# rhofield/rho-tts

Hardware: AMD Instinct MI355X
Metric: audio-sec/wall-sec (RTF) Qwen3-TTS-1.7B batch=32 (higher is better)
Workload: dtype bf16; 1 GPU; Qwen3-TTS-1.7B bf16, batch 32/GPU, 30-s reference clone, 10-word sentences (44 frames each), sampling=top-k 50 T 0.9, seeded synthetic weights; value counts delivered (post-processed) audio; global_batch=32, parallelism=dp1

## Files before the change

rho_tts_amd/csrc/code2wav.hip:

```cpp
#include "model_internal.h"

using namespace rtm;

extern "C" {

int64_t rt_wav_length(rt_model* m, int32_t n_frames) {
    if (!m || n_frames < 0) return -1;
    int64_t L = n_frames;
    for (int i = 0; i < m->cfg.n_upsampling; ++i) L *= m->cfg.upsampling_ratios[i];
    for (int i = 0; i < m->cfg.n_upsample_rates; ++i) L = (L - 1) * m->cfg.upsample_rates[i];
    return L > 0 ? L : 0;
}

int rt_code2wav(rt_model* m, int32_t n_items, int32_t t_max, const int32_t* h_codes, const int32_t* h_n_frames, float* d_wav,
                int64_t wav_stride, int64_t* h_wav_len) {
    if (!m || !h_codes || !h_n_frames || !d_wav || !h_wav_len) return rt_fail(m ? m->ctx : nullptr, RT_ERR_INVALID, "rt_code2wav: null argument");
    rt_ctx* ctx = m->ctx;
    CtxLock g(ctx);
    RT_HIP(ctx, hipSetDevice(ctx->device));
    if (!m->finalized) return rt_fail(ctx, RT_ERR_STATE, "rt_code2wav: model not finalized");
    const rt_model_config& c = m->cfg;
    const int B = n_items, T = t_max, Q = c.num_quantizers, Hc = c.codec_tf.hidden;
    if (B < 1 || B > c.max_batch || T < 1) return rt_fail(ctx, RT_ERR_INVALID, "rt_code2wav: n_items %d / t_max %d out of range", B, T);
    if (T > c.max_codec_frames) return rt_fail(ctx, RT_ERR_LENGTH, "rt_code2wav: length %d frames exceeds max_codec_frames %d", T, c.max_codec_frames);
// ... 77 lines not shown
        RT_TRY(pool_arr(m, (size_t)rows * cout, &xr));
        RT_TRY(planes((size_t)rows * cout, &s1));
        RT_TRY(planes((size_t)rows * cout, &s2));
        {
            GemmA a; a.ptr = s_in.hi; a.ptr_lo = s_in.lo; a.split = 1; a.M = (int64_t)B * (Tc - 1); a.Cin = cin; a.taps = 2; a.tap_stride = 1; a.tap_offset = 0;
            a.rows_out = (int)(Tc - 1); a.rows_in = (int)Tc;
            GemmEpi e; e.bias = VEC(m, bn + ".tconv_b"); e.out_f32 = xr; e.out2_hi = s1.hi; e.out2_lo = s1.lo;
            e.snake2_a = m->xvec[bn + ".u0.a1"]; e.snake2_ib = m->xvec[bn + ".u0.ib1"];
            e.ldc = (int64_t)r * cout;
            RT_TRY(launch_gemm(ctx, a, PW(m, bn + ".tconv"), e));
        }
        for (int j = 0; j < 3; ++j) {
            const std::string u = bn + ".u" + std::to_string(j);
            const int dil = j == 0 ? 1 : (j == 1 ? 3 : 9);
            GemmA a; a.ptr = s1.hi; a.ptr_lo = s1.lo; a.split = 1; a.M = rows; a.Cin = cout; a.taps = 7; a.tap_stride = dil; a.tap_offset = -6 * dil;
            a.rows_out = (int)To; a.rows_in = (int)To;
            GemmEpi e; e.bias = VEC(m, u + ".c1_b"); e.act = ACT_SNAKE; e.snake_a = VEC(m, u + ".a2"); e.snake_ib = VEC(m, u + ".ib2");
            e.out_hi = s2.hi; e.out_lo = s2.lo; e.ldc = cout;
            GemmA a2; a2.ptr = s2.hi; a2.ptr_lo = s2.lo; a2.split = 1; a2.M = rows; a2.Cin = cout;
            GemmEpi e2; e2.bias = VEC(m, u + ".c2_b"); e2.residual = xr; e2.out_f32 = xr; e2.out2_hi = s1.hi; e2.out2_lo = s1.lo; e2.ldc = cout;
            if (j < 2) { e2.snake2_a = VEC(m, bn + ".u" + std::to_string(j + 1) + ".a1"); e2.snake2_ib = VEC(m, bn + ".u" + std::to_string(j + 1) + ".ib1"); }
            else if (i + 1 < c.n_upsample_rates) { e2.snake2_a = VEC(m, "codec.b" + std::to_string(i + 1) + ".sa"); e2.snake2_ib = VEC(m, "codec.b" + std::to_string(i + 1) + ".sib"); }
            else { e2.snake2_a = VEC(m, "codec.fin_a"); e2.snake2_ib = VEC(m, "codec.fin_ib"); }
            if (conv_pair_fusable(a, PW(m, u + ".c1"), e, PW(m, u + ".c2"))) {
                e2.out2_hi = s2.hi; e2.out2_lo = s2.lo;
                RT_TRY(launch_gemm(ctx, a, PW(m, u + ".c1"), e, &PW(m, u + ".c2"), &e2));
                std::swap(s1, s2);
            } else {
                RT_TRY(launch_gemm(ctx, a, PW(m, u + ".c1"), e));
                RT_TRY(launch_gemm(ctx, a2, PW(m, u + ".c2"), e2));
            }
        }
        s_in = s1;
        Tc = To;
    }
    float* wav_tmp = nullptr;
    RT_TRY(pool_arr(m, (size_t)B * Tc, &wav_tmp));
    {
        const int cl = m->dec_ch.back();
        GemmA a; a.ptr = s_in.hi; a.ptr_lo = s_in.lo; a.split = 1; a.M = (int64_t)B * Tc; a.Cin = cl; a.taps = 7; a.tap_stride = 1; a.tap_offset = -6;
        a.rows_out = (int)Tc; a.rows_in = (int)Tc;
        if (launch_final_conv_ok(cl) && g_final_conv) {
            RT_TRY(launch_final_conv(ctx, s_in.hi, s_in.lo, B, (int)Tc, cl, VEC(m, "codec.fin_wv"), VEC(m, "codec.fin_b"), wav_tmp));
        } else {
            GemmEpi e; e.bias = VEC(m, "codec.fin_b"); e.act = ACT_CLAMP1; e.out_f32 = wav_tmp; e.ldc = 1;
            RT_TRY(launch_gemm(ctx, a, PW(m, "codec.fin_w"), e));
        }
    }
    RT_HIP(ctx, hipMemcpy2DAsync(d_wav, (size_t)wav_stride * 4, wav_tmp, (size_t)Tc * 4, (size_t)Tc * 4, B, hipMemcpyDeviceToDevice, ctx->stream));
    RT_HIP(ctx, hipStreamSynchronize(ctx->stream));
    for (int b = 0; b < B; ++b) h_wav_len[b] = rt_wav_length(m, h_n_frames[b]);
    pool_release_all(m);
    return RT_OK;
}
}
```

rho_tts_amd/csrc/debug.hip:

```cpp
#include <algorithm>
#include <vector>

#include "kernels.h"

namespace {
__global__ void k_touch(float* p, int n) {
    const int i = blockIdx.x * blockDim.x + threadIdx.x;
    if (i < n) p[i] = p[i] * 1.0001f + 1.0f;
}
template <int MODE>
__global__ void k_bench_barrier(unsigned* bar, int n, float* buf) {
    const int i = blockIdx.x * blockDim.x + threadIdx.x;
    const int j = (i + blockDim.x) % (gridDim.x * blockDim.x);
    float acc = buf[i];
    for (int e = 1; e <= n; ++e) {
        if (MODE == 2) st_agent(buf + i, acc + 1.0f); else buf[i] = acc + 1.0f;
        if (!grid_barrier<MODE>(bar, gridDim.x, (unsigned)e, 1u << 20)) return;
        acc = MODE == 2 ? ld_agent(buf + j) : buf[j];
        if (acc != (float)e && i == 0) bar[2] = 1u;
    }
    buf[i] = acc;
}
template <int P>
__global__ void k_bench_pair(unsigned* flags, int n, float* buf, unsigned* bar) {
// ... 284 lines not shown
int rt_debug_sample(rt_ctx* ctx, const float* d_logits, int32_t M, int32_t V, const rt_sampling* sp, uint64_t seed, int32_t frame,
                    int32_t group, int32_t suppress_from, int32_t allow_token, uint8_t* d_seen, int32_t* d_out) {
    if (!ctx || !d_logits || !sp || !d_out || M < 1) return rt_fail(ctx, RT_ERR_INVALID, "rt_debug_sample: null argument");
    CtxLock g(ctx);
    RT_HIP(ctx, hipSetDevice(ctx->device));
    int64_t* items = nullptr;
    RT_HIP(ctx, hipMalloc((void**)&items, (size_t)M * 8));
    hipLaunchKernelGGL(k_iota64, dim3((M + 255) / 256), dim3(256), 0, ctx->stream, items, M);
    SampleArgs a{};
    a.logits = d_logits; a.n_slabs = 1; a.M = M; a.V = V;
    a.do_sample = sp->do_sample; a.temperature = sp->temperature; a.top_k = sp->top_k; a.top_p = sp->top_p; a.rep_penalty = sp->repetition_penalty;
    a.seen = d_seen; a.suppress_from = suppress_from; a.allow_token = allow_token; a.seed = seed; a.item_ids = items; a.frame = frame; a.group = group;
    a.forced = nullptr; a.out = d_out; a.out_stride = 1; a.eos_token = -1; a.eos_flag = nullptr; a.logits_copy = nullptr;
    a.frame_ptr = nullptr; a.seed_ptr = nullptr; a.stamps = nullptr;
    int rc = launch_sample(ctx, a);
    (void)hipStreamSynchronize(ctx->stream);
    (void)hipFree(items);
    return rc;
}

int rt_debug_tune(int32_t skinny_variant, int32_t skinny_waves_per_cu) {
    std::unique_lock<std::shared_mutex> all(g_tune_mu);
    if (g_runs_in_flight.load() > 0) return RT_ERR_STATE;
    if (skinny_variant >= 2800) { g_pair_attn = skinny_variant - 2800; return RT_OK; }
    if (skinny_variant >= 2700) { g_frame_inc_fold = skinny_variant - 2700; return RT_OK; }
    if (skinny_variant >= 2600) { g_conv_unroll = skinny_variant - 2600; return RT_OK; }
    if (skinny_variant >= 2400) { g_col_silu_x = skinny_variant - 2400; return RT_OK; }
    if (skinny_variant >= 2300) { g_col_rows16 = skinny_variant - 2300; return RT_OK; }
    if (skinny_variant >= 2200) { g_prefill_attn_mfma = skinny_variant - 2200; return RT_OK; }
    if (skinny_variant >= 2100) { g_fuse_conv = skinny_variant - 2100; return RT_OK; }
    if (skinny_variant >= 2000) { g_col_max_rows = std::min(64, std::max(1, skinny_variant - 2000)); return RT_OK; }
    if (skinny_variant >= 1900) { g_prefill_mid = skinny_variant - 1900; return RT_OK; }
    if (skinny_variant >= 1800) { g_conv_tall = skinny_variant - 1800; return RT_OK; }
    if (skinny_variant >= 1700) { g_handover_every = std::max(1, skinny_variant - 1700); return RT_OK; }
    if (skinny_variant >= 1600) { g_col_split4 = skinny_variant - 1600; return RT_OK; }
    if (skinny_variant >= 1500) { g_attn_mfma = skinny_variant - 1500; return RT_OK; }
    if (skinny_variant >= 1400) { g_eos_check_every = std::max(1, skinny_variant - 1400); return RT_OK; }
    if (skinny_variant >= 1300) { g_sync_parts = skinny_variant - 1300; return RT_OK; }
    if (skinny_variant >= 1200) { g_conv_win = skinny_variant - 1200; return RT_OK; }
    if (skinny_variant >= 1100) { g_final_conv = skinny_variant - 1100; return RT_OK; }
    if (skinny_variant >= 1000) { g_xcd_order = skinny_variant - 1000; return RT_OK; }
    if (skinny_variant >= 900) { g_prefill_fill = skinny_variant - 900; return RT_OK; }
    if (skinny_variant >= 800) { g_fuse_sample_embed = skinny_variant - 800; return RT_OK; }
    if (skinny_variant >= 700) { g_col_rows64 = skinny_variant - 700; return RT_OK; }
    if (skinny_variant >= 600) { g_tile96 = skinny_variant - 600; return RT_OK; }
    if (skinny_variant >= 500) { g_col_split = skinny_variant - 500; return RT_OK; }
// ... 288 lines not shown
```

rho_tts_amd/csrc/gemm.hip:

```cpp
#include <hip/hip_ext.h>

#include "kernels.h"

namespace {

typedef __attribute__((ext_vector_type(8))) __bf16 bf8_t;
typedef __attribute__((ext_vector_type(8))) short s8_t;
typedef __attribute__((ext_vector_type(16))) float f16_t;
typedef __attribute__((ext_vector_type(4))) float f4_t;
typedef __attribute__((ext_vector_type(4))) int i4_t;

__device__ __forceinline__ f16_t mfma32(s8_t a, s8_t b, f16_t c) {
    return __builtin_amdgcn_mfma_f32_32x32x16_bf16(__builtin_bit_cast(bf8_t, a), __builtin_bit_cast(bf8_t, b), c, 0, 0, 0);
}

__device__ __forceinline__ unsigned pack_bf16x2(float lo, float hi) {
    return f32x2_to_bf16x2(lo, hi);
}

__global__ void k_pack_weight(const bf16_t* __restrict__ src, int N, int K, int Np, int Kp, bf16_t* __restrict__ dst) {
    const int KT = Kp / 16;
    const int64_t n_pieces = (int64_t)(Np / 32) * KT * 64;
    for (int64_t p = (int64_t)blockIdx.x * blockDim.x + threadIdx.x; p < n_pieces; p += (int64_t)gridDim.x * blockDim.x) {
        const int lane = (int)(p & 63);
// ... 618 lines not shown
    for (int j = 0; j < PF - 1; ++j) {
        if (it + j < n_it) {
            multiply(j & 1);
            flush();
            stash((j + 1) & 1, rg[j + 1]);
            __syncthreads();
        }
    }
#pragma unroll
    for (int a = 0; a < WM; ++a)
#pragma unroll
        for (int b = 0; b < WN; ++b) {
            const int n = n0 + (wn * WN + b) * 32 + r;
            if (n >= g.N) continue;
#pragma unroll
            for (int i = 0; i < 16; ++i) {
                const int64_t m = m0 + (wm * WM + a) * 32 + (i & 3) + 8 * (i >> 2) + 4 * h;
                if (m < g.M) g.out[m * g.ldc + n] = g.seg_it > 0 ? tot[a][b][i] : acc[a][b][i];
            }
        }
}

template <int WGM, int WGN, int MT, int NTT, bool FUSE = false, int TAPS = 0>
__global__ __launch_bounds__(256, (WGM * MT * 32 > 128) ? 2 : 3) void k_conv_win(TiledArgs g) {
    static_assert(WGM * WGN == 4, "4 waves");
    static_assert(!FUSE || (WGN == 1 && NTT == 3), "the fused 1x1 conv needs every output channel of a row in one wave");
    constexpr int BMT = WGM * MT * 32;
    constexpr int WIN_ROWS = BMT + 64;
    constexpr int NP = (WIN_ROWS * 4 + 255) / 256;
    constexpr int BNT = WGN * NTT * 32;
    constexpr int PLANE = WIN_ROWS * 64;
    constexpr int F_ROWB = NTT * 32 * 2 + 16;
    constexpr int F_WAVE = 2 * 32 * F_ROWB;
    constexpr int LDS_BYTES = (FUSE && 4 * F_WAVE > 2 * 2 * PLANE) ? 4 * F_WAVE : 2 * 2 * PLANE;
    __shared__ __attribute__((aligned(16))) unsigned char lds[LDS_BYTES];
    const int tid = threadIdx.x, lane = tid & 63, w = tid >> 6;
    const int wm = w / WGN, wn = w % WGN;
    const int r = lane & 31, h = lane >> 5;
    int64_t rt = blockIdx.x;
    int ct = blockIdx.y;
    if (g.xcd_order) {
        const int64_t L = (int64_t)blockIdx.y * gridDim.x + blockIdx.x;
        const int xcd = (int)(L & 7);
        const int64_t j = L >> 3;
        ct = (int)(j % gridDim.y);
        rt = (j / gridDim.y) * 8 + xcd;
        if (rt * BMT >= g.a.M) return;
    }
    const int64_t m0 = rt * BMT;
    const int n0 = ct * BNT;
    const int taps = TAPS > 0 ? TAPS : g.a.taps, stride = g.a.tap_stride, Cin = g.a.Cin;
    const int halo = (taps - 1) * stride, WR = BMT + halo, n_cc = Cin >> 5;
    const bf16_t* __restrict__ hi = reinterpret_cast<const bf16_t*>(g.a.ptr);
    const bf16_t* __restrict__ lo = reinterpret_cast<const bf16_t*>(g.a.ptr_lo);

    const int64_t first_row = m0 - halo > 0 ? m0 - halo : 0;
    const int skip = (int)(first_row - (m0 - halo));
// ... 33 lines not shown
    for (int nt = 0; nt < NTT; ++nt) b_off[nt] = nt_base + nt < g.NT ? (unsigned)(((nt_base + nt) * g.KT * 64 + lane) * 16) : 0x80000000u;
    auto load_b = [&](int tap, int cc, s8_t (&b)[NTT][2]) {
        const int t_k0 = (tap * Cin + cc * 32) >> 4;
#pragma unroll
        for (int nt = 0; nt < NTT; ++nt)
#pragma unroll
            for (int kk = 0; kk < 2; ++kk) b[nt][kk] = __builtin_bit_cast(s8_t, __builtin_amdgcn_raw_buffer_load_b128(rs_w, b_off[nt], (t_k0 + kk) * 1024, 0));
    };
    int t_row[MT];
#pragma unroll
    for (int mt = 0; mt < MT; ++mt) {
        const int64_t m = m0 + (wm * MT + mt) * 32 + r;
        t_row[mt] = (int)(m % g.a.rows_out);
    }

    f16_t acc[MT][NTT];
#pragma unroll
    for (int a = 0; a < MT; ++a)
#pragma unroll
        for (int b = 0; b < NTT; ++b)
#pragma unroll
            for (int i = 0; i < 16; ++i) acc[a][b][i] = 0.f;

    s8_t ra[NP], rl[NP], rb[NTT][2], rb_next[NTT][2];
    load_win(0, ra, rl);
    load_b(0, 0, rb);
    store_win(0, ra, rl);
    __syncthreads();
    for (int cc = 0; cc < n_cc; ++cc) {
        const int buf = cc & 1;
        const bool more = cc + 1 < n_cc;
        if (more) load_win(cc + 1, ra, rl);
#pragma unroll
        for (int tap = 0; tap < (TAPS > 0 ? TAPS : taps); ++tap) {
            const bool last = tap + 1 == taps;
            if (!last) load_b(tap + 1, cc, rb_next);
            else if (more) load_b(0, cc + 1, rb_next);
            const int reach = (taps - 1 - tap) * stride;
            s8_t fa[MT][2], fl[MT][2];
#pragma unroll
            for (int mt = 0; mt < MT; ++mt) {
                const int wrow = t_row[mt] >= reach ? (wm * MT + mt) * 32 + r + tap * stride : WIN_ROWS - 1;
#pragma unroll
                for (int kk = 0; kk < 2; ++kk) {
                    fa[mt][kk] = *reinterpret_cast<const s8_t*>(lds + buf * 2 * PLANE + lds_a_off(wrow, kk * 2 + h));
                    fl[mt][kk] = *reinterpret_cast<const s8_t*>(lds + buf * 2 * PLANE + PLANE + lds_a_off(wrow, kk * 2 + h));
                }
            }
#pragma unroll
            for (int kk = 0; kk < 2; ++kk)
#pragma unroll
                for (int mt = 0; mt < MT; ++mt)
#pragma unroll
                    for (int nt = 0; nt < NTT; ++nt) {
                        acc[mt][nt] = mfma32(fa[mt][kk], rb[nt][kk], acc[mt][nt]);
                        acc[mt][nt] = mfma32(fl[mt][kk], rb[nt][kk], acc[mt][nt]);
                    }
            if (!last || more) {
#pragma unroll
                for (int nt = 0; nt < NTT; ++nt)
#pragma unroll
                    for (int kk = 0; kk < 2; ++kk) rb[nt][kk] = rb_next[nt][kk];
            }
        }
        if (more) store_win(buf ^ 1, ra, rl);
        __syncthreads();
    }
    if constexpr (!FUSE) {
        tile_epilogue<MT, NTT>(g, acc, m0, n0, wm, wn, r, h);
    } else {
        unsigned char* my = lds + w * F_WAVE;
        const GemmEpi& e = g.e;
        const __amdgpu_buffer_rsrc_t rs_w2 = __builtin_amdgcn_make_buffer_rsrc((void*)g.Wp2, 0, (unsigned)((int64_t)g.NT2 * g.KT2 * 1024), 0x00020000);
        float f_bias[NTT], f_sa[NTT], f_sib[NTT];
        {
            const float* bp = e.bias ? e.bias : e.snake_a;
#pragma unroll
            for (int nt = 0; nt < NTT; ++nt) {
                const int n = nt * 32 + r;
                f_bias[nt] = bp[n];
                f_sa[nt] = e.snake_a[n];
                f_sib[nt] = e.snake_ib[n];
            }
#pragma unroll
            for (int nt = 0; nt < NTT; ++nt)
                if (!e.bias) f_bias[nt] = 0.f;
        }
        auto load_b2 = [&](int k2, s8_t (&b)[NTT]) {
#pragma unroll
            for (int nt = 0; nt < NTT; ++nt)
                b[nt] = __builtin_bit_cast(s8_t, __builtin_amdgcn_raw_buffer_load_b128(rs_w2, (unsigned)(((nt * g.KT2 + k2) * 64 + lane) * 16), 0, 0));
        };
#pragma unroll
        for (int mt = 0; mt < MT; ++mt) {
            s8_t b2[2][NTT];
            load_b2(0, b2[0]);
#pragma unroll
            for (int nt = 0; nt < NTT; ++nt) {
                const int n = nt * 32 + r;
                const float bias = f_bias[nt], sa = f_sa[nt], sib = f_sib[nt];
#pragma unroll
                for (int i = 0; i < 16; ++i) {
                    float v = acc[mt][nt][i] + bias;
                    const float sn = __sinf(v * sa);
                    v = v + sib * sn * sn;
                    const bf16_t hi = f32_to_bf16(v);
                    const bf16_t lo = f32_to_bf16(v - bf16_to_f32(hi));
                    const int row = (i & 3) + 8 * (i >> 2) + 4 * h;
                    *reinterpret_cast<bf16_t*>(my + row * F_ROWB + n * 2) = hi;
                    *reinterpret_cast<bf16_t*>(my + 32 * F_ROWB + row * F_ROWB + n * 2) = lo;
                }
            }
            f16_t acc2[1][NTT];
#pragma unroll
            for (int nt = 0; nt < NTT; ++nt)
#pragma unroll
                for (int i = 0; i < 16; ++i) acc2[0][nt][i] = 0.f;
#pragma unroll
            for (int k2 = 0; k2 < NTT * 2; ++k2) {
                if (k2 + 1 < NTT * 2) load_b2(k2 + 1, b2[(k2 + 1) & 1]);
                const s8_t a_hi = *reinterpret_cast<const s8_t*>(my + r * F_ROWB + (k2 * 16 + h * 8) * 2);
                const s8_t a_lo = *reinterpret_cast<const s8_t*>(my + 32 * F_ROWB + r * F_ROWB + (k2 * 16 + h * 8) * 2);
#pragma unroll
                for (int nt = 0; nt < NTT; ++nt) {
                    acc2[0][nt] = mfma32(a_hi, b2[k2 & 1][nt], acc2[0][nt]);
                    acc2[0][nt] = mfma32(a_lo, b2[k2 & 1][nt], acc2[0][nt]);
                }
            }
            tile_epilogue_e<1, NTT>(g.e2, g.a.M, g.N2, acc2, m0, 0, wm * MT + mt, 0, r, h);
        }
    }
}

}

size_t packed_bytes(int N, int K) {
    const size_t Np = (size_t)(N + 31) / 32 * 32, Kp = (size_t)(K + 15) / 16 * 16;
    return Np * Kp * 2;
}

size_t packed16_bytes(int N, int K) { return (size_t)((N + 15) / 16 * 16) * K * 2; }

int launch_pack_weight16(rt_ctx* ctx, const bf16_t* d_src, int N, int K, bf16_t* d_dst, PackedW* out) {
    if (K % 32) return rt_fail(ctx, RT_ERR_INVALID, "pack16: K=%d must be a multiple of 32", K);
    const int Np = (N + 15) / 16 * 16;
    const int64_t pieces = (int64_t)(Np / 16) * (K / 32) * 64;
    int64_t blocks = (pieces + 255) / 256;
    if (blocks > 4096) blocks = 4096;
    hipLaunchKernelGGL(k_pack_weight16, dim3((unsigned)blocks), dim3(256), 0, ctx->stream, d_src, N, K, Np, d_dst);
// ... 85 lines not shown

rt_knob g_prefill_mid{1};
bool gemm_mid_shape_ok(const PackedW& w) { return g_prefill_mid && w.K % MID_BK == 0 && w.K >= 128 && w.Kp == w.K; }
bool gemm_mid_ok(int M, const PackedW& w) { return gemm_mid_shape_ok(w) && M > 64 && M <= 1024; }
int launch_gemm_mid(rt_ctx* ctx, const bf16_t* A, int M, const PackedW& w, float* out, int64_t ldc) {
    if (!gemm_mid_ok(M, w)) return rt_fail(ctx, RT_ERR_INVALID, "gemm_mid: M=%d K=%d outside its range", M, w.K);
    MidArgs g{A, w.data, out, M, w.N, w.K, w.Np / 32, w.Kp / 16, ldc, 0};
    const int S = skinny_pick_split(M, w.N, w.K, ctx->n_cu);
    if (S > 1) {
        if ((g.KT / S) % (MID_BK / 16)) return rt_fail(ctx, RT_ERR_STATE, "gemm_mid: K segments of %d k-tiles are not whole 64-deep steps (K=%d, split %d)", g.KT / S, w.K, S);
        g.seg_it = (g.KT / S) / (MID_BK / 16);
    }
    const bool big = g_prefill_mid == 1 ? (int64_t)((M + 127) / 128) * ((w.N + 63) / 64) >= 3 * ctx->n_cu : g_prefill_mid == 3;
    const int bm = big ? 128 : 64;
    const int n_rt = (M + bm - 1) / bm, n_ct = (w.N + 63) / 64;
    dim3 grid(8 * ((n_ct + 7) / 8) * n_rt);
    if (big) hipLaunchKernelGGL((k_gemm_mid<2, 1, 4>), grid, dim3(256), 0, ctx->stream, g);
    else hipLaunchKernelGGL((k_gemm_mid<1, 1, 6>), grid, dim3(256), 0, ctx->stream, g);
    RT_HIP(ctx, hipGetLastError());
    return RT_OK;
}

rt_knob g_fuse_conv{1};

bool conv_pair_fusable(const GemmA& a, const PackedW& w, const GemmEpi& e, const PackedW& w2) {
    return g_fuse_conv && g_conv_win && g_tile96 && w.N == 96 && w2.N == 96 && w2.K == 96 && w2.Kp == 96 && e.act == ACT_SNAKE && a.split && !a.is_f32 && a.ptr_lo && a.taps >= 2 &&
           a.Cin % 32 == 0 && a.rows_out > 0 && a.rows_in == a.rows_out && a.tap_offset == -(a.taps - 1) * a.tap_stride && (a.taps - 1) * a.tap_stride <= 63 &&
           a.M % a.rows_out == 0;
}

int launch_gemm(rt_ctx* ctx, const GemmA& a, const PackedW& w, const GemmEpi& e, const PackedW* w2, const GemmEpi* e2) {
    if (a.M <= 0) return RT_OK;
    if (a.Cin % 8 || (int64_t)a.Cin * a.taps != w.K)
        return rt_fail(ctx, RT_ERR_INVALID, "gemm: A has taps=%d Cin=%d but W has K=%d", a.taps, a.Cin, w.K);
    if (e.split_k < 1 || (e.split_k > 1 && !e.out_f32)) return rt_fail(ctx, RT_ERR_INVALID, "gemm: bad split_k");
    TiledArgs g;
    g.a = a;
    g.Wp = w.data;
    g.N = w.N; g.K = w.K; g.NT = w.Np / 32; g.KT = w.Kp / 16;
    g.e = e;
    int per = (g.KT + e.split_k - 1) / e.split_k;
    per = (per + 1) / 2 * 2;
    g.kt_per_split = per;
    const bool narrow = g_tile96 && e.split_k == 1 && w.N % 96 == 0 && w.N % 128 != 0;
    const bool conv_win = g_conv_win && a.split && !a.is_f32 && a.ptr_lo && a.taps >= 2 && a.Cin % 32 == 0 && a.rows_out > 0 && a.rows_in == a.rows_out &&
        a.tap_offset == -(a.taps - 1) * a.tap_stride && (a.taps - 1) * a.tap_stride <= 63 && e.split_k == 1 && a.M % a.rows_out == 0;
    const bool tall = conv_win && narrow && (g_conv_tall == 2 || (g_conv_tall == 1 && a.M >= 256 * 1024));
    const int bm = tall ? 256 : BM;
    const int64_t my = (a.M + bm - 1) / bm;
    if (my > 0x7fffffff) return rt_fail(ctx, RT_ERR_LENGTH, "gemm: length %lld rows too large", (long long)a.M);
    const int bn = narrow ? 96 : BN;
    const int ny = (w.N + bn - 1) / bn;
    g.xcd_order = (g_xcd_order && e.split_k == 1 && ny > 1 && my >= 64) ? 1 : 0;
    dim3 grid((unsigned)(g.xcd_order ? (my + 7) / 8 * 8 : my), ny, e.split_k);
    if (a.split && !a.is_f32 && !a.ptr_lo) return rt_fail(ctx, RT_ERR_INVALID, "gemm: split precision needs an f32 A operand or a low plane");
    if ((e.out_hi && !e.out_lo) || (e.out2_hi && (!e.out2_lo || (e.act2 != ACT_ELU && (!e.snake2_a || !e.snake2_ib)))) ||
        ((e.out_hi || e.out2_hi) && e.split_k > 1))
        return rt_fail(ctx, RT_ERR_INVALID, "gemm: incomplete hi/lo plane output");
    if (w2) {
        if (!e2 || !conv_win || !narrow || ny != 1 || w.N != 96 || w2->N != 96 || w2->K != 96 || e.act != ACT_SNAKE || !e.snake_a || !e.snake_ib ||
            e2->split_k != 1 || e2->ldc < 96)
            return rt_fail(ctx, RT_ERR_INVALID, "gemm: this conv pair cannot be fused (96 channels, k > 1 conv with SnakeBeta, then a 96 x 96 1x1 conv)");
        g.Wp2 = w2->data; g.NT2 = w2->Np / 32; g.KT2 = w2->Kp / 16; g.N2 = w2->N; g.e2 = *e2;
        const bool t7f = a.taps == 7 && g_conv_unroll;
        if (tall && t7f) hipLaunchKernelGGL((k_conv_win<4, 1, 2, 3, true, 7>), grid, dim3(256), 0, ctx->stream, g);
        else if (tall) hipLaunchKernelGGL((k_conv_win<4, 1, 2, 3, true>), grid, dim3(256), 0, ctx->stream, g);
        else hipLaunchKernelGGL((k_conv_win<4, 1, 1, 3, true>), grid, dim3(256), 0, ctx->stream, g);
        RT_HIP(ctx, hipGetLastError());
        return RT_OK;
    }
    if (conv_win) {
        const bool t7 = a.taps == 7 && g_conv_unroll;
        if (tall && t7) hipLaunchKernelGGL((k_conv_win<4, 1, 2, 3, false, 7>), grid, dim3(256), 0, ctx->stream, g);
        else if (tall) hipLaunchKernelGGL((k_conv_win<4, 1, 2, 3>), grid, dim3(256), 0, ctx->stream, g);
        else if (narrow) hipLaunchKernelGGL((k_conv_win<4, 1, 1, 3>), grid, dim3(256), 0, ctx->stream, g);
        else if (t7) hipLaunchKernelGGL((k_conv_win<2, 2, 2, 2, false, 7>), grid, dim3(256), 0, ctx->stream, g);
        else hipLaunchKernelGGL((k_conv_win<2, 2, 2, 2>), grid, dim3(256), 0, ctx->stream, g);
        RT_HIP(ctx, hipGetLastError());
        return RT_OK;
    }
#define RT_TILED(AF, SP)                                                                                          \
    do {                                                                                                          \
        if (narrow) hipLaunchKernelGGL((k_gemm_tiled<AF, SP, 4, 1, 1, 3>), grid, dim3(256), 0, ctx->stream, g);   \
        else hipLaunchKernelGGL((k_gemm_tiled<AF, SP, 2, 2, 2, 2>), grid, dim3(256), 0, ctx->stream, g);          \
    } while (0)
    if (a.split && !a.is_f32) RT_TILED(false, true);
    else if (a.split) RT_TILED(true, true);
// ... 7 lines not shown
```

rho_tts_amd/csrc/kernels.h:

```cpp
#pragma once
#include "common.h"

struct PackedW {
    const bf16_t* data = nullptr;
    int N = 0, K = 0;
    int Np = 0, Kp = 0;
    size_t bytes() const { return (size_t)Np * Kp * 2; }
    const bf16_t* data16 = nullptr;
    int Np16 = 0;
};

struct GemmA {
    const void* ptr = nullptr;
    const void* ptr_lo = nullptr;
    int is_f32 = 0;
    int split = 0;
    int64_t M = 0;
    int Cin = 0;
    int taps = 1;
    int tap_stride = 1;
    int tap_offset = 0;
    int rows_out = 0;
    int rows_in = 0;
};
// ... 9 lines not shown
    int act = ACT_NONE;
    const float* snake_a = nullptr;
    const float* snake_ib = nullptr;
    bf16_t* out2_bf16 = nullptr;
    float* out2_f32 = nullptr;
    bf16_t* out_hi = nullptr;
    bf16_t* out_lo = nullptr;
    bf16_t* out2_hi = nullptr;
    bf16_t* out2_lo = nullptr;
    const float* snake2_a = nullptr;
    const float* snake2_ib = nullptr;
    int act2 = ACT_SNAKE;
    int64_t ldc = 0;
    int split_k = 1;
};

size_t packed_bytes(int N, int K);
int launch_pack_weight(rt_ctx* ctx, const bf16_t* d_src, int N, int K, bf16_t* d_dst, PackedW* out);
size_t packed16_bytes(int N, int K);
int launch_pack_weight16(rt_ctx* ctx, const bf16_t* d_src, int N, int K, bf16_t* d_dst, PackedW* out);
int launch_gemm(rt_ctx* ctx, const GemmA& a, const PackedW& w, const GemmEpi& e, const PackedW* w2 = nullptr, const GemmEpi* e2 = nullptr);
bool conv_pair_fusable(const GemmA& a, const PackedW& w, const GemmEpi& e, const PackedW& w2);
extern rt_knob g_fuse_conv;
extern rt_knob g_prefill_mid;
bool gemm_mid_ok(int M, const PackedW& w);
bool gemm_mid_shape_ok(const PackedW& w);
int launch_gemm_mid(rt_ctx* ctx, const bf16_t* A, int M, const PackedW& w, float* out, int64_t ldc);
int launch_gemm_skinny(rt_ctx* ctx, const bf16_t* d_a, int M, const PackedW& w, float* d_out, int64_t ldc, int split_k,
                       hipEvent_t ev_start = nullptr, hipEvent_t ev_stop = nullptr, int64_t slab_stride = 0);
int skinny_pick_split(int M, int N, int K, int n_cu);
extern rt_knob g_decode_col;
extern rt_knob g_use_graph;
extern rt_knob g_pred_nt;
extern rt_knob g_decode_lanes;
extern rt_knob g_sync_parts;
extern rt_knob g_eos_check_every;
extern rt_knob g_handover_every;
extern rt_knob g_conv_tall;
extern rt_knob g_col_max_rows;
extern rt_knob g_tile96;
extern rt_knob g_conv_win;
extern rt_knob g_conv_unroll;
extern rt_knob g_final_conv;
extern rt_knob g_xcd_order;
extern rt_knob g_prefill_fill;
extern rt_knob g_pair_attn;
// ... 137 lines not shown
    float* logits_copy;
    const int32_t* frame_ptr;
    const int32_t* frame_off;
    int64_t out_fs, eos_fs, forced_fs, copy_fs;
    int eos_live, min_frames;
    long long* stamps;
    const float* emb_table;
    int emb_H;
    const float* emb_norm_w;
    float* emb_rowsq;
    int emb_rowsq_n;
    float* emb_x_tiled;
    bf16_t* emb_a_tiled;
};
int launch_sample(rt_ctx* ctx, const SampleArgs& a);


int launch_dwconv_ln(rt_ctx* ctx, const float* x, int B, int T, int C, const float* w , const float* b,
                     const float* ln_w, const float* ln_b, float eps, float* out_f32);
int launch_code_embed_mean(rt_ctx* ctx, const bf16_t* table, int codebook, int Q, int H, const int32_t* codes ,
                           int64_t rows, float* out_f32);

bool launch_final_conv_ok(int C);
int launch_final_conv(rt_ctx* ctx, const bf16_t* hi, const bf16_t* lo, int B, int T, int C, const float* w, const float* bias, float* wav);
int launch_f32_to_bf16(rt_ctx* ctx, const float* x, int64_t n, bf16_t* out);

int launch_enc_conv0(rt_ctx* ctx, const float* pcm, int64_t T, int C, int k, const float* w , const float* bias, float* x,
                     bf16_t* hi, bf16_t* lo);
int launch_rvq(rt_ctx* ctx, const float* sem, float* aco, int T, int D, int K, int Q, const float* const* d_cbT, int32_t* codes);
int launch_stats_pool(rt_ctx* ctx, const float* x, int T, int C, float* out);
int launch_gemv_f32(rt_ctx* ctx, const float* W, const float* b, const float* x, int N, int K, int relu, float* y);
```

rho_tts_amd/csrc/rowops.hip:

```cpp
#include "kernels.h"

namespace {

typedef __attribute__((ext_vector_type(4))) float f4_t;

__device__ __forceinline__ float block_sum_f32(float v, float* sh) {
    v = wave_sum_f32(v);
    const int w = threadIdx.x >> 6, nw = (blockDim.x + 63) >> 6;
    __syncthreads();
    if ((threadIdx.x & 63) == 0) sh[w] = v;
    __syncthreads();
    float t = 0.f;
    for (int i = 0; i < nw; ++i) t += sh[i];
    return t;
}

__global__ __launch_bounds__(256) void k_add_rmsnorm(float* __restrict__ x, int H, const float* __restrict__ slabs, int n_slabs,
                                                     int64_t slab_stride, const float* __restrict__ slab_bias,
                                                     const float* __restrict__ scale, const float* __restrict__ w, float eps,
                                                     bf16_t* __restrict__ out_bf16, float* __restrict__ out_f32) {
    __shared__ float sh[4];
    constexpr int MAXV = 8;
    const int64_t row = blockIdx.x;
    const int nv = H >> 2;
// ... 373 lines not shown
    for (int c = threadIdx.x; c < C; c += 256) { const float dlt = row[c] - mean; s2 += dlt * dlt; }
    const float var = block_sum_f32(s2, sh) / (float)C;
    const float inv = rsqrtf(var + eps);
    for (int c = threadIdx.x; c < C; c += 256) out[r * C + c] = (row[c] - mean) * inv * lw[c] + lb[c];
}

__global__ __launch_bounds__(256) void k_code_embed_mean(const bf16_t* __restrict__ table, int codebook, int Q, int H,
                                                         const int32_t* __restrict__ codes, float* __restrict__ out) {
    const int64_t r = blockIdx.x;
    const float inv = 1.f / (float)Q;
    for (int i = threadIdx.x; i < H; i += 256) {
        float v = 0.f;
        for (int q = 0; q < Q; ++q) {
            int c = codes[r * Q + q];
            c = c < 0 ? 0 : (c >= codebook ? codebook - 1 : c);
            v += bf16_to_f32(table[((int64_t)q * codebook + c) * H + i]);
        }
        out[r * H + i] = v * inv;
    }
}


__global__ __launch_bounds__(256) void k_final_conv(const bf16_t* __restrict__ hi, const bf16_t* __restrict__ lo, int T, int C,
                                                    const float* __restrict__ w, const float* __restrict__ bias, float* __restrict__ wav) {
    extern __shared__ float sm[];
    const int stride = C + 1;
    float* tile = sm;
    float* wt = sm + 134 * stride;
    const int b = blockIdx.y, t0 = blockIdx.x * 128, tid = threadIdx.x;
    for (int i = tid; i < 7 * C; i += 256) wt[i] = w[i];
    const int C8 = C >> 3;
    constexpr int IT = 7;
    const int n_items = 134 * C8;
    for (int base = 0; base < n_items; base += 256 * IT) {
        uint4 h[IT], l[IT];
#pragma unroll
        for (int u = 0; u < IT; ++u) {
            int idx = base + u * 256 + tid;
            idx = idx < n_items ? idx : n_items - 1;
            const int row = idx / C8, c = (idx - row * C8) * 8;
            int t = t0 - 6 + row;
            t = t < 0 ? 0 : (t < T ? t : T - 1);
            const int64_t o = ((int64_t)b * T + t) * C + c;
            h[u] = *reinterpret_cast<const uint4*>(hi + o);
            l[u] = *reinterpret_cast<const uint4*>(lo + o);
        }
#pragma unroll
// ... 2 lines not shown
            idx = idx < n_items ? idx : n_items - 1;
            const int row = idx / C8, c = (idx - row * C8) * 8, t = t0 - 6 + row;
            const bool in = t >= 0 && t < T;
            const unsigned hw[4] = {h[u].x, h[u].y, h[u].z, h[u].w}, lw[4] = {l[u].x, l[u].y, l[u].z, l[u].w};
#pragma unroll
            for (int e = 0; e < 4; ++e) {
                const float v0 = __uint_as_float(hw[e] << 16) + __uint_as_float(lw[e] << 16);
                const float v1 = __uint_as_float(hw[e] & 0xffff0000u) + __uint_as_float(lw[e] & 0xffff0000u);
                tile[row * stride + c + 2 * e] = in ? v0 : 0.f;
                tile[row * stride + c + 2 * e + 1] = in ? v1 : 0.f;
            }
        }
    }
    __syncthreads();
    const int s = tid >> 1, half = tid & 1, ch = C >> 1;
    float acc = 0.f;
    for (int k = 0; k < 7; ++k) {
        const float* x = tile + (s + k) * stride + half * ch;
        const float* ww = wt + k * C + half * ch;
        for (int c = 0; c < ch; ++c) acc += x[c] * ww[c];
    }
    acc += __shfl_xor(acc, 1, 64);
    const int t = t0 + s;
    if (half == 0 && t < T) wav[(int64_t)b * T + t] = fminf(1.f, fmaxf(-1.f, acc + bias[0]));
}

__global__ void k_f32_to_bf16(const float* __restrict__ x, int64_t n, bf16_t* __restrict__ out) {
    for (int64_t i = (int64_t)blockIdx.x * blockDim.x + threadIdx.x; i < n; i += (int64_t)gridDim.x * blockDim.x)
        out[i] = f32_to_bf16(x[i]);
}

inline unsigned grid_for(int64_t total, int block = 256) {
    int64_t b = (total + block - 1) / block;
    if (b > 8192) b = 8192;
    if (b < 1) b = 1;
    return (unsigned)b;
}

}

int launch_add_rmsnorm(rt_ctx* ctx, float* x, int M, int H, const float* slabs, int n_slabs, const float* slab_bias,
                       const float* scale, const float* w, float eps, bf16_t* out_bf16, float* out_f32) {
    if (M <= 0) return RT_OK;
    if (H % 4 || H > 8192) return rt_fail(ctx, RT_ERR_UNSUPPORTED, "rmsnorm: hidden size %d unsupported (multiple of 4, <= 8192)", H);
    const int64_t st = (int64_t)M * H;
    if (H == 1024) hipLaunchKernelGGL(k_add_rmsnorm_v<1>, dim3(M), dim3(256), 0, ctx->stream, x, slabs, n_slabs, st, slab_bias, scale, w, eps, out_bf16, out_f32);
    else if (H == 2048) hipLaunchKernelGGL(k_add_rmsnorm_v<2>, dim3(M), dim3(256), 0, ctx->stream, x, slabs, n_slabs, st, slab_bias, scale, w, eps, out_bf16, out_f32);
// ... 88 lines not shown
    return RT_OK;
}


int launch_dwconv_ln(rt_ctx* ctx, const float* x, int B, int T, int C, const float* w, const float* b, const float* ln_w,
                     const float* ln_b, float eps, float* out_f32) {
    const int64_t rows = (int64_t)B * T;
    if (rows <= 0) return RT_OK;
    hipLaunchKernelGGL(k_dwconv_ln, dim3((unsigned)rows), dim3(256), C * sizeof(float), ctx->stream, x, T, C, w, b, ln_w, ln_b, eps, out_f32);
    RT_HIP(ctx, hipGetLastError());
    return RT_OK;
}

int launch_code_embed_mean(rt_ctx* ctx, const bf16_t* table, int codebook, int Q, int H, const int32_t* codes, int64_t rows, float* out_f32) {
    if (rows <= 0) return RT_OK;
    hipLaunchKernelGGL(k_code_embed_mean, dim3((unsigned)rows), dim3(256), 0, ctx->stream, table, codebook, Q, H, codes, out_f32);
    RT_HIP(ctx, hipGetLastError());
    return RT_OK;
}


bool launch_final_conv_ok(int C) { return C % 16 == 0 && (size_t)(134 * (C + 1) + 7 * C) * 4 <= 64 * 1024; }

int launch_final_conv(rt_ctx* ctx, const bf16_t* hi, const bf16_t* lo, int B, int T, int C, const float* w, const float* bias, float* wav) {
    if (B <= 0 || T <= 0) return RT_OK;
    if (!launch_final_conv_ok(C)) return rt_fail(ctx, RT_ERR_UNSUPPORTED, "final conv: %d channels do not fit the LDS window", C);
    const size_t lds = (size_t)(134 * (C + 1) + 7 * C) * 4;
    hipLaunchKernelGGL(k_final_conv, dim3((T + 127) / 128, B), dim3(256), lds, ctx->stream, hi, lo, T, C, w, bias, wav);
    RT_HIP(ctx, hipGetLastError());
    return RT_OK;
}

int launch_f32_to_bf16(rt_ctx* ctx, const float* x, int64_t n, bf16_t* out) {
    if (n <= 0) return RT_OK;
    hipLaunchKernelGGL(k_f32_to_bf16, dim3(grid_for(n)), dim3(256), 0, ctx->stream, x, n, out);
    RT_HIP(ctx, hipGetLastError());
    return RT_OK;
}
```

Measured before the change: 564.9 audio-s/s.

## Fuse 192-channel codec conv pairs and write final waveform directly

Extends the fused k=7 conv + SnakeBeta + 1x1 conv kernel to 192-channel decoder blocks, staging weights in double-buffered LDS and splitting the second GEMM's staging into 96-column halves. The codec's final residual unit skips writing the unused fp32 residual stream, and the final conv writes straight into the strided output buffer instead of a temp plus a 2D memcpy. This removes intermediate global round-trips and one copy in the vocoder, at the cost of higher LDS and register use (lower occupancy bound) for the new kernel variant.

```diff
diff --git a/rho_tts_amd/csrc/code2wav.hip b/rho_tts_amd/csrc/code2wav.hip
--- a/rho_tts_amd/csrc/code2wav.hip
+++ b/rho_tts_amd/csrc/code2wav.hip
@@ -123,6 +123,7 @@
             if (j < 2) { e2.snake2_a = VEC(m, bn + ".u" + std::to_string(j + 1) + ".a1"); e2.snake2_ib = VEC(m, bn + ".u" + std::to_string(j + 1) + ".ib1"); }
             else if (i + 1 < c.n_upsample_rates) { e2.snake2_a = VEC(m, "codec.b" + std::to_string(i + 1) + ".sa"); e2.snake2_ib = VEC(m, "codec.b" + std::to_string(i + 1) + ".sib"); }
             else { e2.snake2_a = VEC(m, "codec.fin_a"); e2.snake2_ib = VEC(m, "codec.fin_ib"); }
+            if (j == 2 && g_c2w_lean) e2.out_f32 = nullptr;
             if (conv_pair_fusable(a, PW(m, u + ".c1"), e, PW(m, u + ".c2"))) {
                 e2.out2_hi = s2.hi; e2.out2_lo = s2.lo;
                 RT_TRY(launch_gemm(ctx, a, PW(m, u + ".c1"), e, &PW(m, u + ".c2"), &e2));
@@ -135,20 +136,25 @@
         s_in = s1;
         Tc = To;
     }
-    float* wav_tmp = nullptr;
-    RT_TRY(pool_arr(m, (size_t)B * Tc, &wav_tmp));
     {
         const int cl = m->dec_ch.back();
-        GemmA a; a.ptr = s_in.hi; a.ptr_lo = s_in.lo; a.split = 1; a.M = (int64_t)B * Tc; a.Cin = cl; a.taps = 7; a.tap_stride = 1; a.tap_offset = -6;
-        a.rows_out = (int)Tc; a.rows_in = (int)Tc;
-        if (launch_final_conv_ok(cl) && g_final_conv) {
-            RT_TRY(launch_final_conv(ctx, s_in.hi, s_in.lo, B, (int)Tc, cl, VEC(m, "codec.fin_wv"), VEC(m, "codec.fin_b"), wav_tmp));
+        const bool own = launch_final_conv_ok(cl) && g_final_conv;
+        if (own && g_c2w_lean) {
+            RT_TRY(launch_final_conv(ctx, s_in.hi, s_in.lo, B, (int)Tc, cl, VEC(m, "codec.fin_wv"), VEC(m, "codec.fin_b"), d_wav, wav_stride));
         } else {
-            GemmEpi e; e.bias = VEC(m, "codec.fin_b"); e.act = ACT_CLAMP1; e.out_f32 = wav_tmp; e.ldc = 1;
-            RT_TRY(launch_gemm(ctx, a, PW(m, "codec.fin_w"), e));
+            float* wav_tmp = nullptr;
+            RT_TRY(pool_arr(m, (size_t)B * Tc, &wav_tmp));
+            if (own) {
+                RT_TRY(launch_final_conv(ctx, s_in.hi, s_in.lo, B, (int)Tc, cl, VEC(m, "codec.fin_wv"), VEC(m, "codec.fin_b"), wav_tmp, Tc));
+            } else {
+                GemmA a; a.ptr = s_in.hi; a.ptr_lo = s_in.lo; a.split = 1; a.M = (int64_t)B * Tc; a.Cin = cl; a.taps = 7; a.tap_stride = 1; a.tap_offset = -6;
+                a.rows_out = (int)Tc; a.rows_in = (int)Tc;
+                GemmEpi e; e.bias = VEC(m, "codec.fin_b"); e.act = ACT_CLAMP1; e.out_f32 = wav_tmp; e.ldc = 1;
+                RT_TRY(launch_gemm(ctx, a, PW(m, "codec.fin_w"), e));
+            }
+            RT_HIP(ctx, hipMemcpy2DAsync(d_wav, (size_t)wav_stride * 4, wav_tmp, (size_t)Tc * 4, (size_t)Tc * 4, B, hipMemcpyDeviceToDevice, ctx->stream));
         }
     }
-    RT_HIP(ctx, hipMemcpy2DAsync(d_wav, (size_t)wav_stride * 4, wav_tmp, (size_t)Tc * 4, (size_t)Tc * 4, B, hipMemcpyDeviceToDevice, ctx->stream));
     RT_HIP(ctx, hipStreamSynchronize(ctx->stream));
     for (int b = 0; b < B; ++b) h_wav_len[b] = rt_wav_length(m, h_n_frames[b]);
     pool_release_all(m);
diff --git a/rho_tts_amd/csrc/debug.hip b/rho_tts_amd/csrc/debug.hip
--- a/rho_tts_amd/csrc/debug.hip
+++ b/rho_tts_amd/csrc/debug.hip
@@ -330,6 +330,8 @@
 int rt_debug_tune(int32_t skinny_variant, int32_t skinny_waves_per_cu) {
     std::unique_lock<std::shared_mutex> all(g_tune_mu);
     if (g_runs_in_flight.load() > 0) return RT_ERR_STATE;
+    if (skinny_variant >= 3000) { g_fuse_conv192 = skinny_variant - 3000; return RT_OK; }
+    if (skinny_variant >= 2900) { g_c2w_lean = skinny_variant - 2900; return RT_OK; }
     if (skinny_variant >= 2800) { g_pair_attn = skinny_variant - 2800; return RT_OK; }
     if (skinny_variant >= 2700) { g_frame_inc_fold = skinny_variant - 2700; return RT_OK; }
     if (skinny_variant >= 2600) { g_conv_unroll = skinny_variant - 2600; return RT_OK; }
diff --git a/rho_tts_amd/csrc/gemm.hip b/rho_tts_amd/csrc/gemm.hip
--- a/rho_tts_amd/csrc/gemm.hip
+++ b/rho_tts_amd/csrc/gemm.hip
@@ -664,17 +664,22 @@
 }
 
 template <int WGM, int WGN, int MT, int NTT, bool FUSE = false, int TAPS = 0>
-__global__ __launch_bounds__(256, (WGM * MT * 32 > 128) ? 2 : 3) void k_conv_win(TiledArgs g) {
+__global__ __launch_bounds__(256, (WGM * MT * 32 > 128 || NTT > 3) ? 2 : 3) void k_conv_win(TiledArgs g) {
     static_assert(WGM * WGN == 4, "4 waves");
-    static_assert(!FUSE || (WGN == 1 && NTT == 3), "the fused 1x1 conv needs every output channel of a row in one wave");
+    static_assert(!FUSE || (WGN == 1 && (NTT == 3 || (NTT == 6 && MT == 1))), "the fused 1x1 conv needs every output channel of a row in one wave");
+    constexpr bool WLDS = FUSE && NTT == 6;
     constexpr int BMT = WGM * MT * 32;
     constexpr int WIN_ROWS = BMT + 64;
     constexpr int NP = (WIN_ROWS * 4 + 255) / 256;
     constexpr int BNT = WGN * NTT * 32;
     constexpr int PLANE = WIN_ROWS * 64;
-    constexpr int F_ROWB = NTT * 32 * 2 + 16;
+    constexpr int F_ROWB = 96 * 2 + 16;
     constexpr int F_WAVE = 2 * 32 * F_ROWB;
-    constexpr int LDS_BYTES = (FUSE && 4 * F_WAVE > 2 * 2 * PLANE) ? 4 * F_WAVE : 2 * 2 * PLANE;
+    constexpr int W_BUF = NTT * 2 * 1024;
+    constexpr int W_OFF = 2 * 2 * PLANE;
+    constexpr int NWP = NTT * 2 * 64 / 256;
+    constexpr int K_BYTES = 2 * 2 * PLANE + (WLDS ? 2 * W_BUF : 0);
+    constexpr int LDS_BYTES = (FUSE && 4 * F_WAVE > K_BYTES) ? 4 * F_WAVE : K_BYTES;
     __shared__ __attribute__((aligned(16))) unsigned char lds[LDS_BYTES];
     const int tid = threadIdx.x, lane = tid & 63, w = tid >> 6;
     const int wm = w / WGN, wn = w % WGN;
@@ -754,6 +759,68 @@
 #pragma unroll
             for (int i = 0; i < 16; ++i) acc[a][b][i] = 0.f;
 
+    if constexpr (WLDS) {
+        unsigned w_off[NWP];
+#pragma unroll
+        for (int i = 0; i < NWP; ++i) {
+            const int f = w + 4 * i;
+            w_off[i] = (unsigned)((((f >> 1) * g.KT + (f & 1)) * 64 + lane) * 16);
+        }
+        auto load_w = [&](int tap, int cc, s8_t (&q)[NWP]) {
+            const int t_k0 = (tap * Cin + cc * 32) >> 4;
+#pragma unroll
+            for (int i = 0; i < NWP; ++i) q[i] = __builtin_bit_cast(s8_t, __builtin_amdgcn_raw_buffer_load_b128(rs_w, w_off[i], t_k0 * 1024, 0));
+        };
+        auto store_w = [&](int wb, const s8_t (&q)[NWP]) {
+#pragma unroll
+            for (int i = 0; i < NWP; ++i) *reinterpret_cast<s8_t*>(lds + W_OFF + wb * W_BUF + (w + 4 * i) * 1024 + lane * 16) = q[i];
+        };
+        s8_t ra[NP], rl[NP], rw[NWP];
+        load_win(0, ra, rl);
+        load_w(0, 0, rw);
+        store_win(0, ra, rl);
+        store_w(0, rw);
+        __syncthreads();
+        int wb = 0;
+        for (int cc = 0; cc < n_cc; ++cc) {
+            const int buf = cc & 1;
+            const bool more = cc + 1 < n_cc;
+            if (more) load_win(cc + 1, ra, rl);
+#pragma unroll
+            for (int tap = 0; tap < (TAPS > 0 ? TAPS : taps); ++tap) {
+                const bool last = tap + 1 == taps;
+                load_w(last ? 0 : tap + 1, last ? cc + 1 : cc, rw);
+                __builtin_amdgcn_sched_barrier(0);
+                const int reach = (taps - 1 - tap) * stride;
+                s8_t fa[MT][2], fl[MT][2];
+#pragma unroll
+                for (int mt = 0; mt < MT; ++mt) {
+                    const int wrow = t_row[mt] >= reach ? (wm * MT + mt) * 32 + r + tap * stride : WIN_ROWS - 1;
+#pragma unroll
+                    for (int kk = 0; kk < 2; ++kk) {
+                        fa[mt][kk] = *reinterpret_cast<const s8_t*>(lds + buf * 2 * PLANE + lds_a_off(wrow, kk * 2 + h));
+                        fl[mt][kk] = *reinterpret_cast<const s8_t*>(lds + buf * 2 * PLANE + PLANE + lds_a_off(wrow, kk * 2 + h));
+                    }
+                }
+                const unsigned char* wl = lds + W_OFF + wb * W_BUF + lane * 16;
+#pragma unroll
+                for (int kk = 0; kk < 2; ++kk)
+#pragma unroll
+                    for (int nt = 0; nt < NTT; ++nt) {
+                        const s8_t fb = *reinterpret_cast<const s8_t*>(wl + (nt * 2 + kk) * 1024);
+#pragma unroll
+                        for (int mt = 0; mt < MT; ++mt) {
+                            acc[mt][nt] = mfma32(fa[mt][kk], fb, acc[mt][nt]);
+                            acc[mt][nt] = mfma32(fl[mt][kk], fb, acc[mt][nt]);
+                        }
+                    }
+                store_w(wb ^ 1, rw);
+                if (last && more) store_win(buf ^ 1, ra, rl);
+                __syncthreads();
+                wb ^= 1;
+            }
+        }
+    } else {
     s8_t ra[NP], rl[NP], rb[NTT][2], rb_next[NTT][2];
     load_win(0, ra, rl);
     load_b(0, 0, rb);
@@ -798,6 +865,7 @@
         if (more) store_win(buf ^ 1, ra, rl);
         __syncthreads();
     }
+    }
     if constexpr (!FUSE) {
         tile_epilogue<MT, NTT>(g, acc, m0, n0, wm, wn, r, h);
     } else {
@@ -827,36 +895,40 @@
         for (int mt = 0; mt < MT; ++mt) {
             s8_t b2[2][NTT];
             load_b2(0, b2[0]);
-#pragma unroll
-            for (int nt = 0; nt < NTT; ++nt) {
-                const int n = nt * 32 + r;
-                const float bias = f_bias[nt], sa = f_sa[nt], sib = f_sib[nt];
-#pragma unroll
-                for (int i = 0; i < 16; ++i) {
-                    float v = acc[mt][nt][i] + bias;
-                    const float sn = __sinf(v * sa);
-                    v = v + sib * sn * sn;
-                    const bf16_t hi = f32_to_bf16(v);
-                    const bf16_t lo = f32_to_bf16(v - bf16_to_f32(hi));
-                    const int row = (i & 3) + 8 * (i >> 2) + 4 * h;
-                    *reinterpret_cast<bf16_t*>(my + row * F_ROWB + n * 2) = hi;
-                    *reinterpret_cast<bf16_t*>(my + 32 * F_ROWB + row * F_ROWB + n * 2) = lo;
-                }
-            }
             f16_t acc2[1][NTT];
 #pragma unroll
             for (int nt = 0; nt < NTT; ++nt)
 #pragma unroll
                 for (int i = 0; i < 16; ++i) acc2[0][nt][i] = 0.f;
 #pragma unroll
-            for (int k2 = 0; k2 < NTT * 2; ++k2) {
-                if (k2 + 1 < NTT * 2) load_b2(k2 + 1, b2[(k2 + 1) & 1]);
-                const s8_t a_hi = *reinterpret_cast<const s8_t*>(my + r * F_ROWB + (k2 * 16 + h * 8) * 2);
-                const s8_t a_lo = *reinterpret_cast<const s8_t*>(my + 32 * F_ROWB + r * F_ROWB + (k2 * 16 + h * 8) * 2);
-#pragma unroll
-                for (int nt = 0; nt < NTT; ++nt) {
-                    acc2[0][nt] = mfma32(a_hi, b2[k2 & 1][nt], acc2[0][nt]);
-                    acc2[0][nt] = mfma32(a_lo, b2[k2 & 1][nt], acc2[0][nt]);
+            for (int hf = 0; hf < NTT / 3; ++hf) {
+#pragma unroll
+                for (int j = 0; j < 3; ++j) {
+                    const int nt = hf * 3 + j, n = j * 32 + r;
+                    const float bias = f_bias[nt], sa = f_sa[nt], sib = f_sib[nt];
+#pragma unroll
+                    for (int i = 0; i < 16; ++i) {
+                        float v = acc[mt][nt][i] + bias;
+                        const float sn = __sinf(v * sa);
+                        v = v + sib * sn * sn;
+                        const bf16_t hi = f32_to_bf16(v);
+                        const bf16_t lo = f32_to_bf16(v - bf16_to_f32(hi));
+                        const int row = (i & 3) + 8 * (i >> 2) + 4 * h;
+                        *reinterpret_cast<bf16_t*>(my + row * F_ROWB + n * 2) = hi;
+                        *reinterpret_cast<bf16_t*>(my + 32 * F_ROWB + row * F_ROWB + n * 2) = lo;
+                    }
+                }
+#pragma unroll
+                for (int kl = 0; kl < 6; ++kl) {
+                    const int k2 = hf * 6 + kl;
+                    if (k2 + 1 < NTT * 2) load_b2(k2 + 1, b2[(k2 + 1) & 1]);
+                    const s8_t a_hi = *reinterpret_cast<const s8_t*>(my + r * F_ROWB + (kl * 16 + h * 8) * 2);
+                    const s8_t a_lo = *reinterpret_cast<const s8_t*>(my + 32 * F_ROWB + r * F_ROWB + (kl * 16 + h * 8) * 2);
+#pragma unroll
+                    for (int nt = 0; nt < NTT; ++nt) {
+                        acc2[0][nt] = mfma32(a_hi, b2[k2 & 1][nt], acc2[0][nt]);
+                        acc2[0][nt] = mfma32(a_lo, b2[k2 & 1][nt], acc2[0][nt]);
+                    }
                 }
             }
             tile_epilogue_e<1, NTT>(g.e2, g.a.M, g.N2, acc2, m0, 0, wm * MT + mt, 0, r, h);
@@ -988,9 +1060,12 @@
 }
 
 rt_knob g_fuse_conv{1};
+rt_knob g_fuse_conv192{1};
+rt_knob g_c2w_lean{1};
 
 bool conv_pair_fusable(const GemmA& a, const PackedW& w, const GemmEpi& e, const PackedW& w2) {
-    return g_fuse_conv && g_conv_win && g_tile96 && w.N == 96 && w2.N == 96 && w2.K == 96 && w2.Kp == 96 && e.act == ACT_SNAKE && a.split && !a.is_f32 && a.ptr_lo && a.taps >= 2 &&
+    const bool c96 = w.N == 96, c192 = w.N == 192 && g_fuse_conv192 && w.Np == 192 && a.taps == 7 && g_conv_unroll;
+    return g_fuse_conv && g_conv_win && g_tile96 && (c96 || c192) && w2.N == w.N && w2.K == w.N && w2.Kp == w.N && w2.Np == w.N && e.act == ACT_SNAKE && a.split && !a.is_f32 && a.ptr_lo && a.taps >= 2 &&
            a.Cin % 32 == 0 && a.rows_out > 0 && a.rows_in == a.rows_out && a.tap_offset == -(a.taps - 1) * a.tap_stride && (a.taps - 1) * a.tap_stride <= 63 &&
            a.M % a.rows_out == 0;
 }
@@ -1024,11 +1099,20 @@
         ((e.out_hi || e.out2_hi) && e.split_k > 1))
         return rt_fail(ctx, RT_ERR_INVALID, "gemm: incomplete hi/lo plane output");
     if (w2) {
-        if (!e2 || !conv_win || !narrow || ny != 1 || w.N != 96 || w2->N != 96 || w2->K != 96 || e.act != ACT_SNAKE || !e.snake_a || !e.snake_ib ||
-            e2->split_k != 1 || e2->ldc < 96)
-            return rt_fail(ctx, RT_ERR_INVALID, "gemm: this conv pair cannot be fused (96 channels, k > 1 conv with SnakeBeta, then a 96 x 96 1x1 conv)");
+        const bool wide = w.N == 192;
+        if (!e2 || !conv_win || !narrow || (!wide && ny != 1) || (w.N != 96 && !wide) || w.Np != w.N || w2->N != w.N || w2->K != w.N || w2->Np != w.N || w2->Kp != w.N ||
+            e.act != ACT_SNAKE || !e.snake_a || !e.snake_ib || e2->split_k != 1 || e2->ldc < w.N)
+            return rt_fail(ctx, RT_ERR_INVALID, "gemm: this conv pair cannot be fused (96 or 192 channels, k > 1 conv with SnakeBeta, then a 1x1 conv of the same width)");
         g.Wp2 = w2->data; g.NT2 = w2->Np / 32; g.KT2 = w2->Kp / 16; g.N2 = w2->N; g.e2 = *e2;
         const bool t7f = a.taps == 7 && g_conv_unroll;
+        if (wide) {
+            g.xcd_order = 0;
+            const dim3 grid_w((unsigned)((a.M + 127) / 128), 1, 1);
+            if (!t7f) return rt_fail(ctx, RT_ERR_INVALID, "gemm: the fused 192-channel conv pair exists for k = 7 with tap unrolling only");
+            hipLaunchKernelGGL((k_conv_win<4, 1, 1, 6, true, 7>), grid_w, dim3(256), 0, ctx->stream, g);
+            RT_HIP(ctx, hipGetLastError());
+            return RT_OK;
+        }
         if (tall && t7f) hipLaunchKernelGGL((k_conv_win<4, 1, 2, 3, true, 7>), grid, dim3(256), 0, ctx->stream, g);
         else if (tall) hipLaunchKernelGGL((k_conv_win<4, 1, 2, 3, true>), grid, dim3(256), 0, ctx->stream, g);
         else hipLaunchKernelGGL((k_conv_win<4, 1, 1, 3, true>), grid, dim3(256), 0, ctx->stream, g);
diff --git a/rho_tts_amd/csrc/kernels.h b/rho_tts_amd/csrc/kernels.h
--- a/rho_tts_amd/csrc/kernels.h
+++ b/rho_tts_amd/csrc/kernels.h
@@ -55,6 +55,8 @@
 int launch_gemm(rt_ctx* ctx, const GemmA& a, const PackedW& w, const GemmEpi& e, const PackedW* w2 = nullptr, const GemmEpi* e2 = nullptr);
 bool conv_pair_fusable(const GemmA& a, const PackedW& w, const GemmEpi& e, const PackedW& w2);
 extern rt_knob g_fuse_conv;
+extern rt_knob g_fuse_conv192;
+extern rt_knob g_c2w_lean;
 extern rt_knob g_prefill_mid;
 bool gemm_mid_ok(int M, const PackedW& w);
 bool gemm_mid_shape_ok(const PackedW& w);
@@ -238,7 +240,8 @@
                            int64_t rows, float* out_f32);
 
 bool launch_final_conv_ok(int C);
-int launch_final_conv(rt_ctx* ctx, const bf16_t* hi, const bf16_t* lo, int B, int T, int C, const float* w, const float* bias, float* wav);
+int launch_final_conv(rt_ctx* ctx, const bf16_t* hi, const bf16_t* lo, int B, int T, int C, const float* w, const float* bias, float* wav,
+                      int64_t wav_stride);
 int launch_f32_to_bf16(rt_ctx* ctx, const float* x, int64_t n, bf16_t* out);
 
 int launch_enc_conv0(rt_ctx* ctx, const float* pcm, int64_t T, int C, int k, const float* w , const float* bias, float* x,
diff --git a/rho_tts_amd/csrc/rowops.hip b/rho_tts_amd/csrc/rowops.hip
--- a/rho_tts_amd/csrc/rowops.hip
+++ b/rho_tts_amd/csrc/rowops.hip
@@ -419,7 +419,8 @@
 
 
 __global__ __launch_bounds__(256) void k_final_conv(const bf16_t* __restrict__ hi, const bf16_t* __restrict__ lo, int T, int C,
-                                                    const float* __restrict__ w, const float* __restrict__ bias, float* __restrict__ wav) {
+                                                    const float* __restrict__ w, const float* __restrict__ bias, float* __restrict__ wav,
+                                                    int64_t wav_stride) {
     extern __shared__ float sm[];
     const int stride = C + 1;
     float* tile = sm;
@@ -468,7 +469,7 @@
     }
     acc += __shfl_xor(acc, 1, 64);
     const int t = t0 + s;
-    if (half == 0 && t < T) wav[(int64_t)b * T + t] = fminf(1.f, fmaxf(-1.f, acc + bias[0]));
+    if (half == 0 && t < T) wav[(int64_t)b * wav_stride + t] = fminf(1.f, fmaxf(-1.f, acc + bias[0]));
 }
 
 __global__ void k_f32_to_bf16(const float* __restrict__ x, int64_t n, bf16_t* __restrict__ out) {
@@ -603,11 +604,13 @@
 
 bool launch_final_conv_ok(int C) { return C % 16 == 0 && (size_t)(134 * (C + 1) + 7 * C) * 4 <= 64 * 1024; }
 
-int launch_final_conv(rt_ctx* ctx, const bf16_t* hi, const bf16_t* lo, int B, int T, int C, const float* w, const float* bias, float* wav) {
+int launch_final_conv(rt_ctx* ctx, const bf16_t* hi, const bf16_t* lo, int B, int T, int C, const float* w, const float* bias, float* wav,
+                      int64_t wav_stride) {
     if (B <= 0 || T <= 0) return RT_OK;
+    if (wav_stride < T) return rt_fail(ctx, RT_ERR_INVALID, "final conv: wav_stride %lld < %d samples", (long long)wav_stride, T);
     if (!launch_final_conv_ok(C)) return rt_fail(ctx, RT_ERR_UNSUPPORTED, "final conv: %d channels do not fit the LDS window", C);
     const size_t lds = (size_t)(134 * (C + 1) + 7 * C) * 4;
-    hipLaunchKernelGGL(k_final_conv, dim3((T + 127) / 128, B), dim3(256), lds, ctx->stream, hi, lo, T, C, w, bias, wav);
+    hipLaunchKernelGGL(k_final_conv, dim3((T + 127) / 128, B), dim3(256), lds, ctx->stream, hi, lo, T, C, w, bias, wav, wav_stride);
     RT_HIP(ctx, hipGetLastError());
     return RT_OK;
 }
```

Measured after the change: 570.6 audio-s/s, median of 6. 1.0% higher.
